# HyeonwooNoh/RAU_VQA

Measured on AMD Instinct MI355X. Metric: QA-pairs/sec fwd+bwd, Ours_SS 8-step RAU, batch 256, 14x14x512, higher is better.
Workload: dtype f32; 1 GPU; Ours_SS 8-step RAU fwd+bwd, 14x14x512, configs[1]; batch_per_gpu=256, global_batch=256, T=26, feature_map=14x14x512, hops=8, parallelism=dp1, collective=none, hop_weights=SS (x nHop), arithmetic=f32 operands, f32 MFMA accumulate, dropout=train mode, Philox masks per step and rank, launch=eager, 3 streams

## Files before the change

### rau_vqa_amd/csrc/common.h

```cpp
#pragma once
#include <hip/hip_runtime.h>
#include <stdint.h>

namespace rau {

typedef float f32x16 __attribute__((ext_vector_type(16)));
typedef float f32x4 __attribute__((ext_vector_type(4)));

constexpr int kWave = 64;

#define RAU_CHAIN_PRIO() __builtin_amdgcn_s_setprio(3)

__device__ __forceinline__ float wave_sum(float v) {
#pragma unroll
  for (int o = 32; o > 0; o >>= 1) v += __shfl_xor(v, o, 64);
  return v;
}
__device__ __forceinline__ float wave_max(float v) {
#pragma unroll
  for (int o = 32; o > 0; o >>= 1) v = fmaxf(v, __shfl_xor(v, o, 64));
  return v;
}
__device__ __forceinline__ float sigmoidf_(float x) { return 1.0f / (1.0f + expf(-x)); }
__device__ __forceinline__ float tanh_fast(float x) {
  const float ax = fabsf(x), x2 = x * x;
  const float p = x * (1.f + x2 * (-0.33333334f + x2 * (0.13333334f + x2 * -0.053968254f)));
  const float t = 1.f - 2.f / (__expf(2.f * ax) + 1.f);
  return ax < 0.125f ? p : copysignf(t, x);
}

__device__ __forceinline__ uint32_t mask_bit(const uint32_t* __restrict__ bits, size_t e) {
  return (bits[e >> 5] >> (e & 31)) & 1u;
}
__device__ __forceinline__ uint32_t mask_nib(const uint32_t* __restrict__ bits, size_t e) {
  return (bits[e >> 5] >> (e & 31)) & 0xFu;
}

__device__ __forceinline__ int xcd_remap(int id, int nwg) {
  const int xcd = id & 7, q = nwg >> 3, r = nwg & 7;
  const int base = xcd < r ? xcd * (q + 1) : r * (q + 1) + (xcd - r) * q;
  return base + (id >> 3);
}

__device__ __forceinline__ float rb16(float x) { return (float)(__bf16)x; }
__device__ __forceinline__ float4 rb16(const float4& v) {
  return make_float4(rb16(v.x), rb16(v.y), rb16(v.z), rb16(v.w));
}

}
```

### rau_vqa_amd/csrc/kernels.h

```cpp
#pragma once
#include <hip/hip_runtime.h>
#include <stddef.h>
#include <stdint.h>

#include "../../include/rau.h"

namespace rau {

constexpr long kMaxSplits = 4096;
constexpr hipError_t kSplitStateError = hipErrorIllegalState;
void split_ws_register(const float* base, size_t floats);
void split_ws_unregister(const float* base);
bool split_span_ok(const float* slab, long nsplit, size_t per_split_floats);

struct LinMode { int bf16 = 0; int deep = 0; };
struct LinOpts {
  const float* bias = nullptr;
  const float* bias2 = nullptr;
  const float* addend = nullptr;
  long add_rs = 0;
  int accumulate = 0;
  int act = 0;
  const float* ymul = nullptr;
  long y_rs = 0;
// ... 170 lines not shown
size_t att_split_part_floats(int nB, int S);
hipError_t att_fwd_split(hipStream_t st, int nB, int M, int A, int S, const float* P,
                         const float* u, const float* ws, const float* bs, const float* zm,
                         const float* I, const float* qf, float* a, float* jv, float* part,
                         const AttPartials& ap = AttPartials());
hipError_t att_bwd_split(hipStream_t st, int nB, int M, int A, int S, const float* I,
                         const float* dj, const float* a, const float* da_lin, const float* ws,
                         float* T_to_dS, float* dz, float* du, float* dwsp, const float* Psrc,
                         const float* u, float* part, int da_ns = 0, int SL = 0,
                         const float* da_add = nullptr);
int att_max_pitch(bool split, int A, int bwd_waves_hint);
inline bool feat_type_ok(int ft) {
  return ft == RAU_FEAT_F32 || ft == RAU_FEAT_F16 || ft == RAU_FEAT_BF16 || ft == RAU_FEAT_E4M3 ||
         ft == RAU_FEAT_E5M2;
}
inline size_t feat_elem_bytes(int ft) {
  return ft == RAU_FEAT_F32 ? 4 : (ft == RAU_FEAT_E4M3 || ft == RAU_FEAT_E5M2) ? 1 : 2;
}
#define RAU_FEAT_TYPE_LIST "RAU_FEAT_F32 | _F16 | _BF16 | _E4M3 | _E5M2"
hipError_t dropout_features(hipStream_t st, int H, size_t per_hop, const void* X,
                            const uint32_t* mask, float mscale, float* xd, size_t mask_e0 = 0,
                            int SL = 0, int Sp = 0, int ft = RAU_FEAT_F32);
hipError_t dropout_features_gen(hipStream_t st, uint64_t seed, uint32_t site, uint32_t step, float p,
                                const uint64_t* key_dev, int H, size_t per_hop, const void* X,
                                float mscale, void* xd, int b16, int ft = RAU_FEAT_F32);
hipError_t dropout_features_b16(hipStream_t st, int H, size_t per_hop, const void* X,
                                const uint32_t* mask, float mscale, void* xd16, int ft = RAU_FEAT_F32);
hipError_t widen_features(hipStream_t st, size_t rows, int SL, int Sp, const void* X, float* out, int ft);
hipError_t expand_features(hipStream_t st, int nB, size_t map_bytes, const void* table, const int32_t* image_of,
                           void* out);
hipError_t bank_gather(hipStream_t st, int n, size_t map_bytes, const void* bank, int32_t capacity,
                       const int32_t* rows, void* out);
hipError_t narrow_features(hipStream_t st, size_t rows, int SL, int Sp, const float* src, void* out, int ft);
hipError_t colsum_acc(hipStream_t st, int rows, int N, const float* X, long ld, float* dst,
                      float* tmp);
hipError_t ce_fwd(hipStream_t st, int nB, int K, int M, const float* logits,
                  const int32_t* labels, const float* mf, const float* wd, const float* bd,
                  float* dl, float* lossrow, int32_t* argmax, float* dopred,
                  const float* part = nullptr, int nsplit = 0, const float* bias = nullptr,
                  float* logits_out = nullptr,
                  int Bper = 0 );
hipError_t loss_reduce(hipStream_t st, int H, int nB, const float* lossrow, float* losses);
constexpr int kMaxAnswers = 16;
hipError_t ce_set_fwd(hipStream_t st, int nB, int K, int M, const float* logits, const int32_t* ids,
                      const float* w, int G, const float* mf, const float* wd, const float* bd, float* dl,
                      float* lossrow, int32_t* argmax, float* dopred, const float* part = nullptr,
                      int nsplit = 0, const float* bias = nullptr, float* logits_out = nullptr, int Bper = 0);
struct Truth {
  const int32_t* labels = nullptr;
  const int32_t* ids = nullptr;
  const float *w = nullptr, *score = nullptr;
  int G = 0;
  bool present() const { return labels || G > 0; }
};
inline const char* criterion_class(const Truth& t) { return t.G > 0 ? "ce_set_fwd" : "ce_fwd"; }
inline hipError_t criterion_head(hipStream_t st, int nB, int K, int M, const float* logits, const Truth& t,
                                 const float* mf, const float* wd, const float* bd, float* dl, float* lossrow,
                                 int32_t* argmax, float* dopred, const float* part = nullptr, int nsplit = 0,
                                 const float* bias = nullptr, float* logits_out = nullptr, int Bper = 0) {
  if (t.G > 0)
    return ce_set_fwd(st, nB, K, M, logits, t.ids, t.w, t.G, mf, wd, bd, dl, lossrow, argmax, dopred, part, nsplit,
                      bias, logits_out, Bper);
  return ce_fwd(st, nB, K, M, logits, t.labels, mf, wd, bd, dl, lossrow, argmax, dopred, part, nsplit, bias,
                logits_out, Bper);
}
hipError_t select_signal(hipStream_t st, int rows, int Bper, int K, int M, const float* dopred,
                         const int32_t* argmax, const Truth& t, const float* selw_dev, const float* wd, float* s,
                         float* add);
// ... 46 lines not shown
```

### rau_vqa_amd/csrc/kernels.hip

```cpp
#include "common.h"
#include <algorithm>
#include <cstdlib>

#include "kernels.h"
#include "philox.h"

namespace rau {

static inline int grid_for(size_t n, int block = 256, int cap = 256 * 8) {
  size_t g = (n + block - 1) / block;
  if (g > (size_t)cap) g = cap;
  if (g < 1) g = 1;
  return (int)g;
}

__global__ void k_fill_masks(uint64_t seed, uint32_t site, uint32_t step, uint32_t thr,
                             size_t nwords, uint32_t* __restrict__ bits,
                             const uint64_t* __restrict__ key) {
  RAU_CHAIN_PRIO();
  if (key) {
    seed = key[0];
    step = (uint32_t)key[1];
  }
  for (size_t w = blockIdx.x * (size_t)blockDim.x + threadIdx.x; w < nwords;
// ... 1542 lines not shown
  LAUNCH_FT(k_widen_features, ft, dim3(grid_for(rows * Sp / 4)), rows * Sp / 4, X,
            reinterpret_cast<float4*>(out));
  return hipGetLastError();
}
#undef LAUNCH_FT

template <typename V>
__global__ __launch_bounds__(256) void k_expand_features(size_t nvec, const V* __restrict__ table,
                                                         const int32_t* __restrict__ image_of,
                                                         V* __restrict__ out) {
  const int b = blockIdx.y;
  const int ib = __builtin_amdgcn_readfirstlane(image_of[b]);
  const V* src = table + (size_t)ib * nvec;
  V* dst = out + (size_t)b * nvec;
  for (size_t i = blockIdx.x * (size_t)blockDim.x + threadIdx.x; i < nvec; i += (size_t)gridDim.x * blockDim.x)
    dst[i] = src[i];
}
hipError_t expand_features(hipStream_t st, int nB, size_t map_bytes, const void* table, const int32_t* image_of,
                           void* out) {
  if (nB <= 0 || !table || !image_of || !out || map_bytes % 8 != 0) return hipErrorInvalidValue;
  const bool v16 = map_bytes % 16 == 0;
  const size_t nvec = map_bytes / (v16 ? 16 : 8);
  const int slices = (int)std::min<size_t>(16, (nvec + 1023) / 1024);
  const dim3 grid(std::max(slices, 1), nB);
  if (v16)
    hipLaunchKernelGGL(k_expand_features<uint4>, grid, dim3(256), 0, st, nvec, static_cast<const uint4*>(table),
                       image_of, static_cast<uint4*>(out));
  else
    hipLaunchKernelGGL(k_expand_features<uint2>, grid, dim3(256), 0, st, nvec, static_cast<const uint2*>(table),
                       image_of, static_cast<uint2*>(out));
  return hipGetLastError();
}

constexpr int kColChunks = 32;
__global__ void k_colsum_stage1(int rows, int N, const float* __restrict__ X, long ld,
                                float* __restrict__ tmp) {
  RAU_CHAIN_PRIO();
  const int n = blockIdx.x * blockDim.x + threadIdx.x;
  if (n >= N) return;
  const int per = (rows + kColChunks - 1) / kColChunks;
  const int r0 = blockIdx.y * per;
  int r1 = r0 + per;
  if (r1 > rows) r1 = rows;
  float acc = 0.f;
  for (int r = r0; r < r1; ++r) acc += X[(size_t)r * ld + n];
  tmp[(size_t)blockIdx.y * N + n] = acc;
}
__global__ __launch_bounds__(256) void k_colsum_stage1_v4(int rows, int N,
                                                         const float* __restrict__ X, long ld,
                                                         float* __restrict__ tmp) {
  __shared__ float4 part[4][64];
  const int l = threadIdx.x & 63, w = threadIdx.x >> 6;
  const int n = (blockIdx.x * 64 + l) * 4;
  const int per = (rows + kColChunks - 1) / kColChunks;
  const int r0 = blockIdx.y * per;
  int r1 = r0 + per;
  if (r1 > rows) r1 = rows;
  float4 a0 = make_float4(0.f, 0.f, 0.f, 0.f), a1 = a0, a2 = a0, a3 = a0;
  if (n < N) {
    const float* p = X + n;
    int r = r0 + w;
    for (; r + 12 < r1; r += 16) {
      const float4 x0 = *reinterpret_cast<const float4*>(p + (size_t)r * ld);
      const float4 x1 = *reinterpret_cast<const float4*>(p + (size_t)(r + 4) * ld);
      const float4 x2 = *reinterpret_cast<const float4*>(p + (size_t)(r + 8) * ld);
      const float4 x3 = *reinterpret_cast<const float4*>(p + (size_t)(r + 12) * ld);
      a0.x += x0.x; a0.y += x0.y; a0.z += x0.z; a0.w += x0.w;
      a1.x += x1.x; a1.y += x1.y; a1.z += x1.z; a1.w += x1.w;
      a2.x += x2.x; a2.y += x2.y; a2.z += x2.z; a2.w += x2.w;
      a3.x += x3.x; a3.y += x3.y; a3.z += x3.z; a3.w += x3.w;
    }
    for (; r < r1; r += 4) {
      const float4 x0 = *reinterpret_cast<const float4*>(p + (size_t)r * ld);
      a0.x += x0.x; a0.y += x0.y; a0.z += x0.z; a0.w += x0.w;
    }
  }
  float4 a;
  a.x = (a0.x + a1.x) + (a2.x + a3.x);
  a.y = (a0.y + a1.y) + (a2.y + a3.y);
  a.z = (a0.z + a1.z) + (a2.z + a3.z);
  a.w = (a0.w + a1.w) + (a2.w + a3.w);
  part[w][l] = a;
  __syncthreads();
  if (w == 0 && n < N) {
    const float4 b = part[1][l], c = part[2][l], d = part[3][l];
    float4 o;
    o.x = (a.x + b.x) + (c.x + d.x);
    o.y = (a.y + b.y) + (c.y + d.y);
    o.z = (a.z + b.z) + (c.z + d.z);
    o.w = (a.w + b.w) + (c.w + d.w);
    *reinterpret_cast<float4*>(tmp + (size_t)blockIdx.y * N + n) = o;
  }
}
__global__ void k_colsum_stage2(int N, const float* __restrict__ tmp, float* __restrict__ dst) {
  RAU_CHAIN_PRIO();
  const int n = blockIdx.x * blockDim.x + threadIdx.x;
  if (n >= N) return;
  float acc = 0.f;
  for (int c = 0; c < kColChunks; ++c) acc += tmp[(size_t)c * N + n];
  dst[n] += acc;
}
hipError_t colsum_acc(hipStream_t st, int rows, int N, const float* X, long ld, float* dst,
                      float* tmp) {
  const bool vec = (N % 4 == 0) && (ld % 4 == 0) && ((reinterpret_cast<uintptr_t>(X) & 15u) == 0) &&
                   rows >= 4 * kColChunks;
  if (vec)
    hipLaunchKernelGGL(k_colsum_stage1_v4, dim3((N + 255) / 256, kColChunks), dim3(256), 0, st,
                       rows, N, X, ld, tmp);
  else
    hipLaunchKernelGGL(k_colsum_stage1, dim3((N + 63) / 64, kColChunks), dim3(64), 0, st, rows, N,
                       X, ld, tmp);
  hipLaunchKernelGGL(k_colsum_stage2, dim3((N + 63) / 64), dim3(64), 0, st, N, tmp, dst);
  return hipGetLastError();
}

__global__ void k_ce_fwd(int nB, int K, int M, const float* __restrict__ logits,
                         const int32_t* __restrict__ labels, const float* __restrict__ mf,
                         const float* __restrict__ wd, const float* __restrict__ bd,
                         float* __restrict__ dl, float* __restrict__ lossrow,
                         int32_t* __restrict__ argmax, float* __restrict__ dopred,
                         const float* __restrict__ part, int nsplit,
                         const float* __restrict__ bias, float* __restrict__ logits_out,
                         int Bper) {
  RAU_CHAIN_PRIO();
  __shared__ float s_val[4];
  __shared__ int s_idx[4];
  __shared__ float s_sum[4];
  const int b = blockIdx.x;
  const int tid = threadIdx.x, l = tid & 63, w = tid >> 6;
  if (nsplit) {
    for (int k = tid; k < K; k += 256) {
      float v = bias[k];
      for (int sp = 0; sp < nsplit; ++sp) v += part[((size_t)sp * nB + b) * K + k];
      logits_out[(size_t)b * K + k] = v;
    }
    __syncthreads();
    logits = logits_out;
  }
  const float* lg = logits + (size_t)b * K;
  float mx = -INFINITY;
  int ai = 0x7fffffff;
  for (int k = tid; k < K; k += 256) {
    const float v = lg[k];
    if (v > mx) { mx = v; ai = k; }
  }
// ... 369 lines not shown
```

### rau_vqa_amd/csrc/rau_ctx.h

```cpp
#pragma once
#include <hip/hip_runtime.h>

#include <algorithm>
#include <array>
#include <cmath>
#include <cstdarg>
#include <cstdio>
#include <cstdlib>
#include <cstring>
#include <numeric>
#include <string>
#include <vector>

#include "../../include/rau.h"
#include "kernels.h"

using namespace rau;

constexpr int kEncHeadTokens = 4;
constexpr int kEncSideChunks = 4;

__attribute__((visibility("hidden"))) int fail(int code, const char* fmt, ...);
#define HIPC(expr)                                                                        \
  do {                                                                                    \
// ... 47 lines not shown
  int ans_G = 0;
  bool regions = false;
};
struct BatchSlot {
  float* feats = nullptr;
  int32_t *tokens = nullptr, *lens_d = nullptr, *labels_d = nullptr;
  int32_t *utok = nullptr, *ustart = nullptr, *upos = nullptr;
  int32_t* image_of_d = nullptr;
  int32_t* bank_idx_d = nullptr;
  float* feats_h = nullptr;
  int32_t *tokens_h = nullptr, *lens_p = nullptr, *labels_h = nullptr;
  int32_t *utok_h = nullptr, *ustart_h = nullptr, *upos_h = nullptr;
  int32_t* image_of_h = nullptr;
  int32_t* bank_idx_h = nullptr;
  int32_t* ans_ids_d = nullptr;
  float *ans_w_d = nullptr, *ans_score_d = nullptr;
  int32_t* ans_h = nullptr;
  bool ans_pending = false;
  int32_t* nreg_d = nullptr;
  int32_t* nreg_h = nullptr;
  bool reg_pending = false;
  hipEvent_t uploaded = nullptr;
  hipEvent_t consumed = nullptr;
  BatchDesc held;
  bool upload_pending = false, consumed_valid = false;
};

struct StreamWs {
  hipStream_t owner = nullptr;
  float* slab = nullptr;
  size_t floats = 0;
  size_t alloc = 0;
  float* coltmp = nullptr;
};

inline Truth truth_of(const BatchSlot& s) {
  return s.held.have_labels ? Truth{s.labels_d, s.ans_ids_d, s.ans_w_d, s.ans_score_d, s.held.ans_G} : Truth{};
}

struct MergeState {
  bool valid = false;
  Truth truth;
  int slot = 0;
  uint64_t serial = 0, fwd = 0;
  bool merged = false;
  uint64_t pred_fwd = 0;
  bool pred_mc = false;
  bool ready = false;
  float *rowf = nullptr, *out = nullptr, *pred = nullptr, *att = nullptr;
  int32_t *rowi = nullptr, *ans = nullptr, *mc = nullptr;
  size_t mc_cap = 0;
  float* score = nullptr;
  void* topk = nullptr;
  int topk_k = 0;
  void invalidate() { valid = merged = false; truth = Truth{}; }
};

struct rau_ctx {
  rau_config cfg;
  int cap = 0;
  int Q;
  int Sp = 0;
  int bf16 = 0;
  hipStream_t st = nullptr;
  hipStream_t st2 = nullptr;
  hipStream_t st3 = nullptr;
// ... 295 lines not shown
```

### rau_vqa_amd/csrc/rau_ctx.hip

```cpp
#include "rau_ctx.h"

static thread_local char g_err[512] = "";
int fail(int code, const char* fmt, ...) {
  va_list ap;
  va_start(ap, fmt);
  vsnprintf(g_err, sizeof(g_err), fmt, ap);
  va_end(ap);
  return code;
}

static int prof_collect(rau_ctx* ctx) {
  if (ctx->precs.empty()) return 0;
  HIPC(hipStreamSynchronize(ctx->st));
  HIPC(hipStreamSynchronize(ctx->st2));
  HIPC(hipStreamSynchronize(ctx->st3));
  if (ctx->stc) HIPC(hipStreamSynchronize(ctx->stc));
  FILE* tl = nullptr;
  if (const char* p = std::getenv("RAU_PROF_TIMELINE")) tl = std::fopen(p, "a");
  for (auto& r : ctx->precs) {
    float ms = 0.f;
    hipEventElapsedTime(&ms, r.a, r.b);
    if (tl) {
      float t0 = 0.f;
      hipEventElapsedTime(&t0, ctx->precs[0].a, r.a);
// ... 407 lines not shown
  CK(dalloc(ctx, &ctx->losses_d, (size_t)H));
  CK(dalloc(ctx, &ctx->hopw_d, (size_t)2 * H));
  {
    hipError_t eh = hipHostMalloc((void**)&ctx->hopw_h, (size_t)4 * H * sizeof(float), hipHostMallocDefault);
    if (eh != hipSuccess) {
      rau_destroy(ctx);
      return fail(RAU_ERR_NOMEM, "hipHostMalloc(hop weights): %s", hipGetErrorString(eh));
    }
  }
  CK(dalloc(ctx, &ctx->argmax_d, HB));
  CK(dalloc(ctx, &ctx->dpre, HB * M));
  CK(dalloc(ctx, &ctx->dhn, HB * R));
  CK(dalloc(ctx, &ctx->dg4, HB * 4 * R));
  for (int i = 0; i < 2; ++i) {
    CK(dalloc(ctx, &ctx->dcn[i], (size_t)B * R));
    CK(dalloc(ctx, &ctx->dhp[i], (size_t)B * R));
  }
  CK(dalloc(ctx, &ctx->dj, HB * M));
  CK(dalloc(ctx, &ctx->da_lin, (size_t)B * S));
  CK(dalloc(ctx, &ctx->dz, HB * S));
  CK(dalloc(ctx, &ctx->du, HB * A));
  CK(dalloc(ctx, &ctx->dwsp, HB * A));
  CK(dalloc(ctx, &ctx->dZ, HB * M * S));
  CK(dalloc(ctx, &ctx->dqt, HB * M));
  CK(dalloc(ctx, &ctx->dQD, HB * Q));
  CK(dalloc(ctx, &ctx->dq, (size_t)B * Q));
  for (StreamWs* w : stream_ws(ctx)) {
    CK(dalloc(ctx, &w->slab, w->floats));
    w->alloc = w->floats;
    split_ws_register(w->slab, w->floats);
  }
  {
    const int widest = std::max({4 * R, 4 * Rq, K, M, S, A, Q});
    CK(dalloc(ctx, &ctx->ws_side.coltmp, (size_t)32 * widest));
    CK(dalloc(ctx, &ctx->ws_bulk.coltmp, (size_t)32 * widest));
    CK(dalloc(ctx, &ctx->dbi_part, (size_t)H * B * M));
    CK(dalloc(ctx, &ctx->tmpS, (size_t)S));
  }
  CK(dalloc(ctx, &ctx->dG1, TB * 4 * Rq));
  CK(dalloc(ctx, &ctx->dG2, TB * 4 * Rq));
  CK(dalloc(ctx, &ctx->dwe, TB * E));
  for (int L = 0; L < 2; ++L) {
    CK(dalloc(ctx, &ctx->edc[L][0], (size_t)B * Rq));
    CK(dalloc(ctx, &ctx->edc[L][1], (size_t)B * Rq));
  }
  CK(dalloc(ctx, &ctx->dkey, (size_t)2, false));
  CK(dalloc(ctx, &ctx->npart, (size_t)1024));
  CK(dalloc(ctx, &ctx->norms_d, (size_t)4));
#undef CK
  {
    hipError_t es = hipStreamSynchronize(ctx->st);
    if (es != hipSuccess) {
      rau_destroy(ctx);
      return fail(RAU_ERR_DEVICE, "rau_create sync: %s", hipGetErrorString(es));
    }
  }
  *out = ctx;
  return RAU_OK;
}

void rau_destroy(rau_ctx* ctx) {
  if (!ctx) return;
  rau_comm_destroy(ctx);
  if (ctx->st_comm) hipStreamDestroy(ctx->st_comm);
  if (ctx->evC) hipEventDestroy(ctx->evC);
  if (ctx->st) hipStreamSynchronize(ctx->st);
  if (ctx->st2) hipStreamSynchronize(ctx->st2);
  if (ctx->st3) hipStreamSynchronize(ctx->st3);
// ... 849 lines not shown
  const size_t BRq = (size_t)B * Rq;
  ctx->fwd_done = false;

  if (!ctx->capturing) {
    if (int rc = upload_hop_weights(ctx, hop_w, select_w)) return rc;
  }
  if (ctx->dpre_fwd && !sel)
    RUN("scale_hops", 0, (double)H * B * (K + M + R) * 8,
        scale_hops3(st, H, ctx->hopw_d, (size_t)B * K, ctx->dl, (size_t)B * M, ctx->dpre, (size_t)B * R, ctx->dhn));
  else
    RUN("scale_hops", 0, (double)H * B * K * 8, scale_hops(st, H, (size_t)B * K, ctx->hopw_d, ctx->dl));

  int HA = 0;
  for (int h = 0; h < H; ++h)
    if (hop_w[h] != 0.f || (sel && select_w[h] != 0.f)) HA = h + 1;

  const uint32_t* m_mf = mk(RAU_MASK_MF);
  if (sel)
    RUN("select_signal", 0, (double)HA * B * M * 4,
        select_signal(st, HA * B, B, K, M, ctx->dopred, ctx->argmax_d, t, ctx->hopw_d + H, ctx->do_pred.W, ctx->sel_s,
                      ctx->sel_add));
  if (HA > 0 && (!ctx->dpre_fwd || sel)) {
    LinOpts o = lin_opts(ctx, ctx->ws_chain);
    if (sel) { o.addend = ctx->sel_add; o.add_rs = M; }
    o.emask = m_mf;
    o.emask_e0 = 0;
    o.emscale = sc(RAU_MASK_MF);
    RUN("head_dgrad", gflop(HA * B, M, K), 0,
        gemm_nn(st, HA * B, M, K, ctx->dl, K, ctx->cls.W, M, ctx->dpre, M, o));
    const LinOpts o2 = lin_opts(ctx, ctx->ws_chain);
    RUN("head_dgrad", gflop(HA * B, R, M), 0,
        gemm_nn(st, HA * B, R, M, ctx->dpre, M, ctx->lstm_out.W, R, ctx->dhn, R, o2));
  }
  const float* dc_next = nullptr;
  float* dh_part = nullptr;
  int dh_part_ns = 0;
  ctx->ds16_step = ctx->dS16 && !ctx->I_shared && !ctx->att_split && conv_dz_fused_ok(S, M, ctx->bf16);
  struct Ds16Reset { rau_ctx* c; ~Ds16Reset() { c->ds16_step = false; } } ds16_reset{ctx};
  bool dq_side = false;
  int dq_rows_left = HA;
  for (int h = HA - 1; h >= 0; --h) {
    float* dc_out = ctx->dcn[h & 1];
    {
      HopGrad g{};
      g.dl = ctx->dl + (size_t)h * B * K;
      g.dc_next = dc_next;
      g.dh_next = nullptr;
      g.dc_out = dc_out;
      g.dh_out = nullptr;
      g.dpre_ready = 1;
      g.dhn_all = ctx->dhn;
      g.dh_part = dh_part;
      g.dh_part_ns = dh_part_ns;
      g.dh_part_out = &dh_part;
      g.dh_part_ns_out = &dh_part_ns;
      g.ev_conv_ready = (gsz[h] && (seam_mask() & 2)) ? ctx->evK[h] : nullptr;
      g.dh_prev_dead = h == 0;
      if (int rc = hop_backward(ctx, h, ctx->cc + (size_t)h * BR_,
                                ctx->I + (ctx->I_shared ? 0 : (size_t)h * BM_ * S), g))
        return rc;
    }
    dc_next = dc_out;
    if (gsz[h] && h > 0 && side_split(ctx)) {
      const int nh = std::min(h + gsz[h], HA) - h;
      HIPC(hipEventRecord(ctx->evK[h], st));
      HIPC(hipStreamWaitEvent(ctx->st3, ctx->evK[h], 0));
// ... 23 lines not shown
                                 ctx->att_i.W, ctx->dj + hb * M,
                                 ctx->a + hb * S, ctx->I + hb * M * S,
                                 ctx->xd16 ? (float*)((uint16_t*)ctx->dZ + hb * M * S) : ctx->dZ + hb * M * S,
                                 ctx->dbi_part + hb * M, ctx->xd16 ? 1 : 0, ctx->bf16, ctx->ds16_step ? 1 : 0,
                                 chain_bound(ctx) ? 1 : 0));
        else
          RUNS(sb, "conv_att_dgrad", gflop(M, (double)nH * S, A),
               ((double)nH * A * S + 2.0 * nH * M * S) * 4,
               conv_att_dgrad(sb, nH, M, S, A, ctx->T + hb * A * S, ctx->att_i.W, ctx->dj + hb * M,
                              ctx->a + hb * S, ctx->dZ + hb * M * S, ctx->bf16));
        {
          if (ctx->ds16_step)
            RUNS(sb, "conv_att_wgrad", gflop(A, M, (double)nH * S),
                 (double)nH * A * S * 2 + (double)nH * M * S * 4,
                 conv_att_wgrad_ds16(sb, nH, M, S, A, (const uint16_t*)ctx->dS16 + hb * A * S,
                                     ctx->I + hb * M * S, ctx->att_i.dW, slab_b));
          else
          RUNS(sb, "conv_att_wgrad", gflop(A, M, (double)nH * S),
               ((double)nH * A * S + (double)nH * M * S) * 4,
               conv_att_wgrad(sb, nH, M, S, A, ctx->T + hb * A * S, ctx->I + hb * M * S,
                              ctx->att_i.dW, slab_b, ctx->bf16));
        }
        if (ctx->xd16 && dzf)
          RUNS(sb, "conv_embed_wgrad", gflop(M, D, (double)nH * S),
               (double)nH * M * S * 2 + (double)nH * D * S * 2,
               conv_embed_wgrad_b16(sb, nH, D, S, M, (const uint16_t*)ctx->dZ + hb * M * S,
                                    (const uint16_t*)ctx->xd16 + hb * D * S, ctx->i_embed.dW, slab_b));
        else
          RUNS(sb, "conv_embed_wgrad", gflop(M, D, (double)nH * S),
               ((double)nH * M * S * (dzf ? 1 : 2) + (double)nH * D * S) * 4,
               conv_embed_wgrad(sb, nH, D, S, M, ctx->dZ + hb * M * S, ctx->I + hb * M * S,
                                  ctx->xd + hb * D * S, ctx->i_embed.dW, slab_b, ctx->bf16,
                                  ctx->i_embed.db, dzf));
        if (dzf && h == 0)
          RUNS(sb, "colsum", 0, (double)HA * B * M * 4,
               colsum_acc(sb, HA * B, M, ctx->dbi_part, M, ctx->i_embed.db, ctx->ws_bulk.coltmp));
      } else {
        for (int hh2 = 0; hh2 < HA; ++hh2) {
          float* Th2 = ctx->T + (size_t)hh2 * B * A * S;
          float* dZh = ctx->dZ + (size_t)hh2 * BM_ * S;
          RUNS(sb, "conv_att_dgrad", gflop(M, (double)B * S, A), ((double)B * A * S + 2.0 * BM_ * S) * 4,
               conv_att_dgrad(sb, B, M, S, A, Th2, ctx->att_i.W, ctx->dj + (size_t)hh2 * BM_,
                              ctx->a + (size_t)hh2 * BS_, dZh, ctx->bf16));
          RUNS(sb, "conv_att_wgrad", gflop(A, M, (double)B * S), ((double)B * A * S + BM_ * S) * 4,
               conv_att_wgrad(sb, B, M, S, A, Th2, ctx->I, ctx->att_i.dW, slab_b, ctx->bf16));
          RUNS(sb, "conv_embed_wgrad", gflop(M, D, (double)B * S), (BM_ * S + (double)B * D * S) * 4,
               conv_embed_wgrad(sb, B, D, S, M, dZh, ctx->I, ctx->xw, ctx->i_embed.dW, slab_b,
                                ctx->bf16, ctx->i_embed.db));
        }
      }
    }
  }
  {
    const LinOpts o = lin_opts(ctx, ctx->ws_chain);
    if (dq_rows_left > 0)
      RUN("q_proj_dgrad", gflop(dq_rows_left * B, Q, M), 0,
          gemm_nn(st, dq_rows_left * B, Q, M, ctx->dqt, M, ctx->q_proj.W, Q, ctx->dQD, Q, o));
    if (dq_side) HIPC(hipStreamWaitEvent(st, ctx->evDq, 0));
    RUN("dq_reduce", 0, (double)HA * B * Q * 4,
        dq_reduce(st, HA, (size_t)B * Q, ctx->dQD, m_q, sc(RAU_MASK_Q), ctx->dq));
  }
  {
    hipStream_t sb = ctx->st2;
    HIPC(hipEventRecord(ctx->evD, sb));
  }
  HIPC(hipEventRecord(ctx->evW, st));
  static const int wg_env = [] { const char* e = std::getenv("RAU_WG_BULK"); return e ? std::atoi(e) : -1; }();
  const int wg_bulk = side_split(ctx) ? 0 : wg_env >= 0 ? wg_env : (chain_bound(ctx) ? 0 : 1);
  auto mult_wgrads = [&]() -> int {
    const StreamWs& ws = (wg_bulk & 1) ? ctx->ws_bulk : ctx->ws_side;
    hipStream_t sw = ws.owner;
    HIPC(hipStreamWaitEvent(sw, ctx->evW, 0));
    const int rows = HA * B;
    if (rows == 0) {
      HIPC(hipEventRecord(ctx->evM3, sw));
      return 0;
    }
    {
      TnProblem pr[13];
      const int np = mult_wgrad_problems(ctx, pr);
      double fl = 0;
      for (int i = 0; i < np; ++i) fl += gflop(pr[i].M, pr[i].N, rows);
      RUNS(sw, "wgrad_gemm", fl, 0, gemm_tn_group_acc(sw, pr, np, rows, ws.slab, ws.floats, lin_mode(ctx).bf16));
    }
    if (sel)
      RUNS(sw, "select_wgrad", 2.0 * rows * (M + 1), (double)rows * M * 4,
           select_wgrad(sw, rows, M, ctx->sel_s, ctx->mf, ctx->do_pred.dW, ctx->do_pred.db));
    RUNS(sw, "colsum", 0, (double)rows * A * 4, colsum_acc(sw, rows, A, ctx->dwsp, A, ctx->att_score.dW, ws.coltmp));
    HIPC(hipMemsetAsync(ctx->tmpS, 0, S * sizeof(float), sw));
    RUNS(sw, "colsum", 0, (double)rows * S * 4, colsum_acc(sw, rows, SL, ctx->dz, S, ctx->tmpS, ws.coltmp));
    RUNS(sw, "colsum", 0, S * 4.0, colsum_acc(sw, SL, 1, ctx->tmpS, 1, ctx->att_score.db, ws.coltmp));
    RUNS(sw, "colsum", 0, (double)rows * A * 4, colsum_acc(sw, rows, A, ctx->du, A, ctx->att_i.db, ws.coltmp));
    HIPC(hipEventRecord(ctx->evM3, sw));
    return 0;
  };
  if (int rc = mult_wgrads()) return rc;

  if (TL > 0) {
    const int rows = TL * B;
    const size_t G4 = (size_t)B * 4 * Rq;
    auto enc_wgrads = [&](int t_lo, int t_hi, hipEvent_t ev) -> int {
      if (t_hi <= t_lo) return 0;
      const StreamWs& ws = (wg_bulk & 2) ? ctx->ws_bulk : ctx->ws_side;
      hipStream_t sw = ws.owner;
      HIPC(hipEventRecord(ev, st));
      HIPC(hipStreamWaitEvent(sw, ev, 0));
      const size_t r0 = (size_t)t_lo * B;
      const int nr = (t_hi - t_lo) * B;
      TnProblem pr[13];
      const int np = enc_wgrad_problems(ctx, r0, pr);
      double fl = 0;
      for (int i = 0; i < np; ++i) fl += gflop(pr[i].M, pr[i].N, nr);
      RUNS(sw, "wgrad_gemm", fl, 0, gemm_tn_group_acc(sw, pr, np, nr, ws.slab, ws.floats, lin_mode(ctx).bf16));
      return 0;
    };
    const int hi = TL;
    for (int u = TL; u >= 0; --u) {
      const float* Ap[3];
      const float* Wp[3];
      int nb = 0, iq2 = -1, iqx = -1, iq1 = -1;
      if (u >= 1 && u + 1 <= TL) { Ap[nb] = ctx->dG2 + (size_t)u * G4; Wp[nb] = ctx->h2h[1].W; iq2 = nb++; }
      if (u + 1 <= TL) { Ap[nb] = ctx->dG2 + (size_t)u * G4; Wp[nb] = ctx->i2h[1].W; iqx = nb++; }
      if (u + 2 <= TL) { Ap[nb] = ctx->dG1 + (size_t)(u + 1) * G4; Wp[nb] = ctx->h2h[0].W; iq1 = nb++; }
      int nsp = 0;
      if (nb > 0)
// ... 317 lines not shown
```

### rau_vqa_amd/csrc/rau_modules.hip

```cpp
#include "rau_ctx.h"

namespace {

bool aligned16(const void* p) { return (reinterpret_cast<uintptr_t>(p) & 15u) == 0; }

int mod_alloc(rau_ctx* ctx) {
  ctx->mg.valid = false;
  if (ctx->mod_ready) return 0;
  const rau_config& c = ctx->cfg;
  const size_t B = ctx->cap, Q = ctx->Q;
  const size_t wide = std::max<size_t>({(size_t)c.Rq, (size_t)c.R, (size_t)c.M});
#define CK(x) do { if (int rc_ = (x)) return rc_; } while (0)
  CK(dalloc(ctx, &ctx->m_state, (size_t)c.T * B * Q));
  CK(dalloc(ctx, &ctx->m_dstate, (size_t)c.T * B * Q));
  for (int i = 0; i < 4; ++i) CK(dalloc(ctx, &ctx->m_tmp[i], B * wide));
  CK(dalloc(ctx, &ctx->m_dq, (size_t)c.H * B * Q));
  CK(dalloc(ctx, &ctx->m_dc, (size_t)c.H * B * c.R));
  CK(dalloc(ctx, &ctx->m_dh, (size_t)c.H * B * c.R));
  CK(dalloc(ctx, &ctx->m_add, B * c.M));
  CK(dalloc(ctx, &ctx->m_s, B));
  CK(dalloc(ctx, &ctx->m_zero, B * std::max<size_t>(Q, (size_t)c.R)));
  CK(dalloc(ctx, &ctx->m_loss, (size_t)c.H));
  if (ctx->Sp != c.S) {
    CK(dalloc(ctx, &ctx->m_Xp, B * c.D * ctx->Sp));
// ... 317 lines not shown
  const size_t BM_ = (size_t)B * M, BS_ = (size_t)B * S, BR_ = (size_t)B * R;
  if (S != SL) {
    if (!resident) {
      if (int rc = repitch(ctx, ctx->m_Xp, S, X, SL, (size_t)B * D)) return rc;
      X = ctx->m_Xp;
    }
    if (d_attprob) {
      HIPC(hipMemsetAsync(ctx->m_da, 0, BS_ * sizeof(float), st));
      if (int rc = repitch(ctx, ctx->m_da, S, d_attprob, SL, B)) return rc;
      d_attprob = ctx->m_da;
    }
  }
  const float* Ih = ctx->I + (size_t)h * BM_ * S;
  const float* mfh = ctx->mf + (size_t)h * BM_;
  float* Th = ctx->T + (size_t)h * B * A * S;
  float* dZh = ctx->dZ + (size_t)h * BM_ * S;
  const float* xin = m.x ? ctx->xd + (size_t)h * B * D * S : X;

  HopGrad g{};
  g.dl = d_logits;
  g.dc_next = d_c;
  g.dh_next = d_h;
  g.da_out = d_attprob;
  g.dc_out = ctx->m_dc + (size_t)h * BR_;
  g.dh_out = ctx->m_dh + (size_t)h * BR_;
  if (d_do_pred) {
    RUN("dopred_bwd", 0, 0, sigmoid_bwd(st, B, d_do_pred, ctx->dopred + (size_t)h * B, ctx->m_s));
    RUN("dopred_bwd", 0, 0, row_scale(st, B, M, ctx->m_s, nullptr, ctx->do_pred.W, ctx->m_add));
    g.dmf_add = ctx->m_add;
  }
  if (int rc = hop_backward(ctx, h, c_prev, Ih, g)) return rc;
  if (d_do_pred) {
    RUN("dopred_bwd", 0, 0, row_scale(st, B, M, ctx->m_s, mfh, nullptr, ctx->m_add));
    RUN("colsum", 0, 0, colsum_acc(st, B, M, ctx->m_add, M, ctx->do_pred.dW, ctx->ws_side.coltmp));
    RUN("colsum", 0, 0, colsum_acc(st, B, 1, ctx->m_s, 1, ctx->do_pred.db, ctx->ws_side.coltmp));
  }
  RUN("conv_att_dgrad", gflop(M, (double)B * S, A), ((double)B * A * S + 2.0 * BM_ * S) * 4,
      conv_att_dgrad(st, B, M, S, A, Th, ctx->att_i.W, ctx->dj + (size_t)h * BM_,
                     ctx->a + (size_t)h * BS_, dZh, ctx->bf16));
  RUN("conv_att_wgrad", gflop(A, M, (double)B * S), ((double)B * A * S + BM_ * S) * 4,
      conv_att_wgrad(st, B, M, S, A, Th, Ih, ctx->att_i.dW, ctx->ws_bulk.slab, ctx->bf16));
  RUN("conv_embed_wgrad", gflop(M, D, (double)B * S), (BM_ * S + (double)B * D * S) * 4,
      conv_embed_wgrad(st, B, D, S, M, dZh, Ih, xin, ctx->i_embed.dW, ctx->ws_bulk.slab, ctx->bf16,
                       ctx->i_embed.db));
  float* dqo = ctx->m_dq + (size_t)h * B * Q;
  {
    LinOpts o = lin_opts(ctx, ctx->ws_chain);
    o.emask = m.q;
    o.emask_e0 = (size_t)h * B * Q;
    o.emscale = m.s_q;
    RUN("q_proj_dgrad", gflop(B, Q, M), 0,
        gemm_nn(st, B, Q, M, ctx->dqt + (size_t)h * BM_, M, ctx->q_proj.W, Q, dqo, Q, o));
  }
  if (d_X) {
    if (!ctx->m_dX) {
      if (int rc = dalloc(ctx, &ctx->m_dX, (size_t)ctx->cap * D * S)) return rc;
      if (int rc = dalloc(ctx, &ctx->m_dZ, (size_t)ctx->cap * M * S)) return rc;
    }
    RUN("mul_dtanh", 0, BM_ * S * 12.0, mul_dtanh(st, BM_ * S, dZh, Ih, ctx->m_dZ));
    RUN("conv_embed_dgrad", gflop(D, (double)B * S, M), (BM_ * S + (double)B * D * S) * 4,
        conv_embed_dgrad(st, B, D, S, M, ctx->m_dZ, ctx->i_embed.W, ctx->m_dX));
    float* dXo = ctx->m_dX;
    if (S != SL) {
      if (!ctx->m_dXd)
        if (int rc = dalloc(ctx, &ctx->m_dXd, (size_t)ctx->cap * D * SL)) return rc;
      if (int rc = repitch(ctx, ctx->m_dXd, SL, ctx->m_dX, S, (size_t)B * D)) return rc;
      dXo = ctx->m_dXd;
    }
    if (m.x)
      RUN("apply_mask", 0, (double)B * D * SL * 8,
          apply_mask(st, (size_t)B * D * SL, (size_t)B * D * SL, dXo, m.x, m.s_x, dXo,
                     (size_t)h * B * D * SL));
    *d_X = dXo;
  }
  const size_t h4 = (size_t)h * B * 4 * R;
  if (int rc = lin_wgrad(ctx, ctx->cls, d_logits, mfh, M)) return rc;
  if (int rc = lin_wgrad(ctx, ctx->lstm_out, ctx->dpre + (size_t)h * BM_, ctx->hh + (size_t)(h + 1) * BR_, R)) return rc;
  if (int rc = lin_wgrad(ctx, ctx->lstm_i2h, ctx->dg4 + h4, ctx->j + (size_t)h * BM_, M)) return rc;
  if (int rc = lin_wgrad(ctx, ctx->lstm_h2h, ctx->dg4 + h4, h_prev, R)) return rc;
  if (int rc = lin_wgrad(ctx, ctx->feat_attprob, ctx->dj + (size_t)h * BM_, ctx->a + (size_t)h * BS_, S)) return rc;
  if (int rc = lin_wgrad(ctx, ctx->att_mem, ctx->dz + (size_t)h * BS_, h_prev, R, true, S)) return rc;
  if (int rc = lin_wgrad(ctx, ctx->att_q, ctx->du + (size_t)h * B * A, ctx->qf + (size_t)h * BM_, M)) return rc;
  if (int rc = lin_wgrad(ctx, ctx->q_proj, ctx->dqt + (size_t)h * BM_, ctx->qd + (size_t)h * B * Q, Q)) return rc;
  if (int rc = lin_wgrad(ctx, ctx->h_proj, ctx->dqt + (size_t)h * BM_, h_prev, R)) return rc;
  RUN("colsum", 0, (double)B * A * 4,
      colsum_acc(st, B, A, ctx->dwsp + (size_t)h * B * A, A, ctx->att_score.dW, ctx->ws_side.coltmp));
  HIPC(hipMemsetAsync(ctx->tmpS, 0, S * sizeof(float), st));
  RUN("colsum", 0, (double)B * S * 4, colsum_acc(st, B, SL, ctx->dz + (size_t)h * BS_, S, ctx->tmpS, ctx->ws_side.coltmp));
  RUN("colsum", 0, S * 4.0, colsum_acc(st, SL, 1, ctx->tmpS, 1, ctx->att_score.db, ctx->ws_side.coltmp));
  RUN("colsum", 0, (double)B * A * 4,
      colsum_acc(st, B, A, ctx->du + (size_t)h * B * A, A, ctx->att_i.db, ctx->ws_side.coltmp));
  if (d_q) *d_q = dqo;
  if (d_c_prev) *d_c_prev = g.dc_out;
  if (d_h_prev) *d_h_prev = g.dh_out;
  return RAU_OK;
}

static int criterion(rau_ctx* ctx, int h, const float* logits, const Truth& t, float* loss, float scale,
                     float** d_logits) {
  const rau_config& c = ctx->cfg;
  float* dl = ctx->dl + (size_t)h * c.B * c.K;
  RUN(criterion_class(t), 0, (double)c.B * c.K * 12,
      criterion_head(ctx->st, c.B, c.K, c.M, logits, t, nullptr, nullptr, nullptr, dl,
                     ctx->lossrow + (size_t)h * c.B, ctx->argmax_d + (size_t)h * c.B, nullptr));
  if (d_logits) {
    if (scale != 1.f)
      RUN("scale_hops", 0, (double)c.B * c.K * 8, scale_inplace(ctx->st, (size_t)c.B * c.K, scale, dl));
    *d_logits = dl;
    return RAU_OK;
  }
  RUN("loss_reduce", 0, 0, loss_reduce(ctx->st, 1, c.B, ctx->lossrow + (size_t)h * c.B, ctx->m_loss + h));
  if (!loss) return RAU_OK;
  HIPC(hipMemcpyAsync(loss, ctx->m_loss + h, sizeof(float), hipMemcpyDeviceToHost, ctx->st));
  HIPC(hipStreamSynchronize(ctx->st));
  return RAU_OK;
}

int rau_criterion_forward(rau_ctx* ctx, int h, const float* logits, const int32_t* labels_dev, float* loss) {
  NEED(ctx && logits, "null argument");
  NEED(h >= 0 && h < ctx->cfg.H, "rau_criterion_forward: h=%d out of [0,%d)", h, ctx->cfg.H);
  if (int rc = mod_alloc(ctx)) return rc;
  const Truth t = labels_dev ? Truth{labels_dev} : truth_of(cur_batch(ctx));
  if (!t.present()) return fail(RAU_ERR_STATE, "rau_criterion_forward: no labels");
  return criterion(ctx, h, logits, t, loss, 1.f, nullptr);
// ... 32 lines not shown
```

Measured before the change: 27680 QA-pairs/s.

## Fuse two-stage column sum into one kernel with last-block reduction

Result: no change. 27620 QA-pairs/s (-0.2%).

```diff
diff --git a/rau_vqa_amd/csrc/common.h b/rau_vqa_amd/csrc/common.h
--- a/rau_vqa_amd/csrc/common.h
+++ b/rau_vqa_amd/csrc/common.h
@@ -20,6 +20,24 @@
 #pragma unroll
   for (int o = 32; o > 0; o >>= 1) v = fmaxf(v, __shfl_xor(v, o, 64));
   return v;
+}
+__device__ __forceinline__ bool last_arrival(unsigned* cnt, unsigned total, int* s_flag) {
+  asm volatile("s_waitcnt vmcnt(0)" ::: "memory");
+  __syncthreads();
+  if (threadIdx.x == 0) {
+    __builtin_amdgcn_fence(__ATOMIC_RELEASE, "agent");
+    asm volatile("s_waitcnt vmcnt(0)" ::: "memory");
+    const unsigned ticket = __hip_atomic_fetch_add(cnt, 1u, __ATOMIC_RELAXED, __HIP_MEMORY_SCOPE_AGENT);
+    const int last = ticket == total - 1;
+    if (last) {
+      __hip_atomic_store(cnt, 0u, __ATOMIC_RELAXED, __HIP_MEMORY_SCOPE_AGENT);
+      __builtin_amdgcn_fence(__ATOMIC_ACQUIRE, "agent");
+      asm volatile("s_waitcnt vmcnt(0)" ::: "memory");
+    }
+    *s_flag = last;
+  }
+  __syncthreads();
+  return *s_flag != 0;
 }
 __device__ __forceinline__ float sigmoidf_(float x) { return 1.0f / (1.0f + expf(-x)); }
 __device__ __forceinline__ float tanh_fast(float x) {
diff --git a/rau_vqa_amd/csrc/kernels.h b/rau_vqa_amd/csrc/kernels.h
--- a/rau_vqa_amd/csrc/kernels.h
+++ b/rau_vqa_amd/csrc/kernels.h
@@ -226,8 +226,9 @@
 hipError_t bank_gather(hipStream_t st, int n, size_t map_bytes, const void* bank, int32_t capacity,
                        const int32_t* rows, void* out);
 hipError_t narrow_features(hipStream_t st, size_t rows, int SL, int Sp, const float* src, void* out, int ft);
+constexpr int kColChunks = 32;
 hipError_t colsum_acc(hipStream_t st, int rows, int N, const float* X, long ld, float* dst,
-                      float* tmp);
+                      float* tmp, unsigned* cnt, int accumulate = 1);
 hipError_t ce_fwd(hipStream_t st, int nB, int K, int M, const float* logits,
                   const int32_t* labels, const float* mf, const float* wd, const float* bd,
                   float* dl, float* lossrow, int32_t* argmax, float* dopred,
diff --git a/rau_vqa_amd/csrc/kernels.hip b/rau_vqa_amd/csrc/kernels.hip
--- a/rau_vqa_amd/csrc/kernels.hip
+++ b/rau_vqa_amd/csrc/kernels.hip
@@ -1598,85 +1598,77 @@
   return hipGetLastError();
 }
 
-constexpr int kColChunks = 32;
-__global__ void k_colsum_stage1(int rows, int N, const float* __restrict__ X, long ld,
-                                float* __restrict__ tmp) {
-  RAU_CHAIN_PRIO();
-  const int n = blockIdx.x * blockDim.x + threadIdx.x;
-  if (n >= N) return;
+__global__ __launch_bounds__(256) void k_colsum(int rows, int N, const float* __restrict__ X, long ld,
+                                                float* __restrict__ dst, float* __restrict__ tmp,
+                                                unsigned* __restrict__ cnt, int vec, int accumulate) {
+  __shared__ float4 part[4][64];
+  __shared__ int is_last;
+  const int tile = blockIdx.x, chunk = blockIdx.y;
   const int per = (rows + kColChunks - 1) / kColChunks;
-  const int r0 = blockIdx.y * per;
+  const int r0 = chunk * per;
   int r1 = r0 + per;
   if (r1 > rows) r1 = rows;
-  float acc = 0.f;
-  for (int r = r0; r < r1; ++r) acc += X[(size_t)r * ld + n];
-  tmp[(size_t)blockIdx.y * N + n] = acc;
-}
-__global__ __launch_bounds__(256) void k_colsum_stage1_v4(int rows, int N,
-                                                         const float* __restrict__ X, long ld,
-                                                         float* __restrict__ tmp) {
-  __shared__ float4 part[4][64];
-  const int l = threadIdx.x & 63, w = threadIdx.x >> 6;
-  const int n = (blockIdx.x * 64 + l) * 4;
-  const int per = (rows + kColChunks - 1) / kColChunks;
-  const int r0 = blockIdx.y * per;
-  int r1 = r0 + per;
-  if (r1 > rows) r1 = rows;
-  float4 a0 = make_float4(0.f, 0.f, 0.f, 0.f), a1 = a0, a2 = a0, a3 = a0;
-  if (n < N) {
-    const float* p = X + n;
-    int r = r0 + w;
-    for (; r + 12 < r1; r += 16) {
-      const float4 x0 = *reinterpret_cast<const float4*>(p + (size_t)r * ld);
-      const float4 x1 = *reinterpret_cast<const float4*>(p + (size_t)(r + 4) * ld);
-      const float4 x2 = *reinterpret_cast<const float4*>(p + (size_t)(r + 8) * ld);
-      const float4 x3 = *reinterpret_cast<const float4*>(p + (size_t)(r + 12) * ld);
-      a0.x += x0.x; a0.y += x0.y; a0.z += x0.z; a0.w += x0.w;
-      a1.x += x1.x; a1.y += x1.y; a1.z += x1.z; a1.w += x1.w;
-      a2.x += x2.x; a2.y += x2.y; a2.z += x2.z; a2.w += x2.w;
-      a3.x += x3.x; a3.y += x3.y; a3.z += x3.z; a3.w += x3.w;
-    }
-    for (; r < r1; r += 4) {
-      const float4 x0 = *reinterpret_cast<const float4*>(p + (size_t)r * ld);
-      a0.x += x0.x; a0.y += x0.y; a0.z += x0.z; a0.w += x0.w;
-    }
-  }
-  float4 a;
-  a.x = (a0.x + a1.x) + (a2.x + a3.x);
-  a.y = (a0.y + a1.y) + (a2.y + a3.y);
-  a.z = (a0.z + a1.z) + (a2.z + a3.z);
-  a.w = (a0.w + a1.w) + (a2.w + a3.w);
-  part[w][l] = a;
-  __syncthreads();
-  if (w == 0 && n < N) {
-    const float4 b = part[1][l], c = part[2][l], d = part[3][l];
-    float4 o;
-    o.x = (a.x + b.x) + (c.x + d.x);
-    o.y = (a.y + b.y) + (c.y + d.y);
-    o.z = (a.z + b.z) + (c.z + d.z);
-    o.w = (a.w + b.w) + (c.w + d.w);
-    *reinterpret_cast<float4*>(tmp + (size_t)blockIdx.y * N + n) = o;
-  }
-}
-__global__ void k_colsum_stage2(int N, const float* __restrict__ tmp, float* __restrict__ dst) {
-  RAU_CHAIN_PRIO();
-  const int n = blockIdx.x * blockDim.x + threadIdx.x;
-  if (n >= N) return;
-  float acc = 0.f;
-  for (int c = 0; c < kColChunks; ++c) acc += tmp[(size_t)c * N + n];
-  dst[n] += acc;
+  if (vec) {
+    const int l = threadIdx.x & 63, w = threadIdx.x >> 6;
+    const int n = (tile * 64 + l) * 4;
+    float4 a0 = make_float4(0.f, 0.f, 0.f, 0.f), a1 = a0, a2 = a0, a3 = a0;
+    if (n < N) {
+      const float* p = X + n;
+      int r = r0 + w;
+      for (; r + 12 < r1; r += 16) {
+        const float4 x0 = *reinterpret_cast<const float4*>(p + (size_t)r * ld);
+        const float4 x1 = *reinterpret_cast<const float4*>(p + (size_t)(r + 4) * ld);
+        const float4 x2 = *reinterpret_cast<const float4*>(p + (size_t)(r + 8) * ld);
+        const float4 x3 = *reinterpret_cast<const float4*>(p + (size_t)(r + 12) * ld);
+        a0.x += x0.x; a0.y += x0.y; a0.z += x0.z; a0.w += x0.w;
+        a1.x += x1.x; a1.y += x1.y; a1.z += x1.z; a1.w += x1.w;
+        a2.x += x2.x; a2.y += x2.y; a2.z += x2.z; a2.w += x2.w;
+        a3.x += x3.x; a3.y += x3.y; a3.z += x3.z; a3.w += x3.w;
+      }
+      for (; r < r1; r += 4) {
+        const float4 x0 = *reinterpret_cast<const float4*>(p + (size_t)r * ld);
+        a0.x += x0.x; a0.y += x0.y; a0.z += x0.z; a0.w += x0.w;
+      }
+    }
+    float4 a;
+    a.x = (a0.x + a1.x) + (a2.x + a3.x);
+    a.y = (a0.y + a1.y) + (a2.y + a3.y);
+    a.z = (a0.z + a1.z) + (a2.z + a3.z);
+    a.w = (a0.w + a1.w) + (a2.w + a3.w);
+    part[w][l] = a;
+    __syncthreads();
+    if (w == 0 && n < N) {
+      const float4 b = part[1][l], c = part[2][l], d = part[3][l];
+      float4 o;
+      o.x = (a.x + b.x) + (c.x + d.x);
+      o.y = (a.y + b.y) + (c.y + d.y);
+      o.z = (a.z + b.z) + (c.z + d.z);
+      o.w = (a.w + b.w) + (c.w + d.w);
+      *reinterpret_cast<float4*>(tmp + (size_t)chunk * N + n) = o;
+    }
+  } else {
+    const int n = tile * 256 + threadIdx.x;
+    if (n < N) {
+      float acc = 0.f;
+      for (int r = r0; r < r1; ++r) acc += X[(size_t)r * ld + n];
+      tmp[(size_t)chunk * N + n] = acc;
+    }
+  }
+  if (!last_arrival(cnt, gridDim.x * gridDim.y, &is_last)) return;
+  for (int n = threadIdx.x; n < N; n += 256) {
+    float acc = 0.f;
+    for (int c = 0; c < kColChunks; ++c) acc += tmp[(size_t)c * N + n];
+    if (accumulate) dst[n] += acc;
+    else dst[n] = acc;
+  }
 }
 hipError_t colsum_acc(hipStream_t st, int rows, int N, const float* X, long ld, float* dst,
-                      float* tmp) {
-  const bool vec = (N % 4 == 0) && (ld % 4 == 0) && ((reinterpret_cast<uintptr_t>(X) & 15u) == 0) &&
-                   rows >= 4 * kColChunks;
-  if (vec)
-    hipLaunchKernelGGL(k_colsum_stage1_v4, dim3((N + 255) / 256, kColChunks), dim3(256), 0, st,
-                       rows, N, X, ld, tmp);
-  else
-    hipLaunchKernelGGL(k_colsum_stage1, dim3((N + 63) / 64, kColChunks), dim3(64), 0, st, rows, N,
-                       X, ld, tmp);
-  hipLaunchKernelGGL(k_colsum_stage2, dim3((N + 63) / 64), dim3(64), 0, st, N, tmp, dst);
+                      float* tmp, unsigned* cnt, int accumulate) {
+  if (N <= 0) return hipSuccess;
+  const int vec = (N % 4 == 0) && (ld % 4 == 0) && ((reinterpret_cast<uintptr_t>(X) & 15u) == 0) &&
+                  rows >= 4 * kColChunks;
+  hipLaunchKernelGGL(k_colsum, dim3((N + 255) / 256, kColChunks), dim3(256), 0, st, rows, N, X, ld, dst, tmp,
+                     cnt, vec, accumulate);
   return hipGetLastError();
 }
 
diff --git a/rau_vqa_amd/csrc/rau_ctx.h b/rau_vqa_amd/csrc/rau_ctx.h
--- a/rau_vqa_amd/csrc/rau_ctx.h
+++ b/rau_vqa_amd/csrc/rau_ctx.h
@@ -103,6 +103,7 @@
   size_t floats = 0;
   size_t alloc = 0;
   float* coltmp = nullptr;
+  unsigned* colcnt = nullptr;
 };
 
 inline Truth truth_of(const BatchSlot& s) {
diff --git a/rau_vqa_amd/csrc/rau_ctx.hip b/rau_vqa_amd/csrc/rau_ctx.hip
--- a/rau_vqa_amd/csrc/rau_ctx.hip
+++ b/rau_vqa_amd/csrc/rau_ctx.hip
@@ -463,8 +463,12 @@
   }
   {
     const int widest = std::max({4 * R, 4 * Rq, K, M, S, A, Q});
-    CK(dalloc(ctx, &ctx->ws_side.coltmp, (size_t)32 * widest));
-    CK(dalloc(ctx, &ctx->ws_bulk.coltmp, (size_t)32 * widest));
+    for (StreamWs* w : {&ctx->ws_side, &ctx->ws_bulk}) {
+      CK(dalloc(ctx, &w->coltmp, (size_t)kColChunks * widest));
+      float* f = nullptr;
+      CK(dalloc(ctx, &f, 4));
+      w->colcnt = reinterpret_cast<unsigned*>(f);
+    }
     CK(dalloc(ctx, &ctx->dbi_part, (size_t)H * B * M));
     CK(dalloc(ctx, &ctx->tmpS, (size_t)S));
   }
@@ -1380,6 +1384,9 @@
     RUN("head_dgrad", gflop(HA * B, R, M), 0,
         gemm_nn(st, HA * B, R, M, ctx->dpre, M, ctx->lstm_out.W, R, ctx->dhn, R, o2));
   }
+  static const int wg_env = [] { const char* e = std::getenv("RAU_WG_BULK"); return e ? std::atoi(e) : -1; }();
+  const int wg_bulk = side_split(ctx) ? 0 : wg_env >= 0 ? wg_env : (chain_bound(ctx) ? 0 : 1);
+  bool dbi_pending = false;
   const float* dc_next = nullptr;
   float* dh_part = nullptr;
   int dh_part_ns = 0;
@@ -1469,9 +1476,14 @@
                conv_embed_wgrad(sb, nH, D, S, M, ctx->dZ + hb * M * S, ctx->I + hb * M * S,
                                   ctx->xd + hb * D * S, ctx->i_embed.dW, slab_b, ctx->bf16,
                                   ctx->i_embed.db, dzf));
-        if (dzf && h == 0)
-          RUNS(sb, "colsum", 0, (double)HA * B * M * 4,
-               colsum_acc(sb, HA * B, M, ctx->dbi_part, M, ctx->i_embed.db, ctx->ws_bulk.coltmp));
+        if (dzf && h == 0) {
+          if (wg_bulk & 1)
+            dbi_pending = true;
+          else
+            RUNS(sb, "colsum", 0, (double)HA * B * M * 4,
+                 colsum_acc(sb, HA * B, M, ctx->dbi_part, M, ctx->i_embed.db, ctx->ws_bulk.coltmp,
+                            ctx->ws_bulk.colcnt));
+        }
       } else {
         for (int hh2 = 0; hh2 < HA; ++hh2) {
           float* Th2 = ctx->T + (size_t)hh2 * B * A * S;
@@ -1502,8 +1514,6 @@
     HIPC(hipEventRecord(ctx->evD, sb));
   }
   HIPC(hipEventRecord(ctx->evW, st));
-  static const int wg_env = [] { const char* e = std::getenv("RAU_WG_BULK"); return e ? std::atoi(e) : -1; }();
-  const int wg_bulk = side_split(ctx) ? 0 : wg_env >= 0 ? wg_env : (chain_bound(ctx) ? 0 : 1);
   auto mult_wgrads = [&]() -> int {
     const StreamWs& ws = (wg_bulk & 1) ? ctx->ws_bulk : ctx->ws_side;
     hipStream_t sw = ws.owner;
@@ -1513,6 +1523,16 @@
       HIPC(hipEventRecord(ctx->evM3, sw));
       return 0;
     }
+    if (dbi_pending)
+      RUNS(sw, "colsum", 0, (double)rows * M * 4,
+           colsum_acc(sw, rows, M, ctx->dbi_part, M, ctx->i_embed.db, ws.coltmp, ws.colcnt));
+    RUNS(sw, "colsum", 0, (double)rows * A * 4,
+         colsum_acc(sw, rows, A, ctx->dwsp, A, ctx->att_score.dW, ws.coltmp, ws.colcnt));
+    RUNS(sw, "colsum", 0, (double)rows * S * 4,
+         colsum_acc(sw, rows, SL, ctx->dz, S, ctx->tmpS, ws.coltmp, ws.colcnt, 0));
+    RUNS(sw, "colsum", 0, S * 4.0, colsum_acc(sw, SL, 1, ctx->tmpS, 1, ctx->att_score.db, ws.coltmp, ws.colcnt));
+    RUNS(sw, "colsum", 0, (double)rows * A * 4,
+         colsum_acc(sw, rows, A, ctx->du, A, ctx->att_i.db, ws.coltmp, ws.colcnt));
     {
       TnProblem pr[13];
       const int np = mult_wgrad_problems(ctx, pr);
@@ -1523,11 +1543,6 @@
     if (sel)
       RUNS(sw, "select_wgrad", 2.0 * rows * (M + 1), (double)rows * M * 4,
            select_wgrad(sw, rows, M, ctx->sel_s, ctx->mf, ctx->do_pred.dW, ctx->do_pred.db));
-    RUNS(sw, "colsum", 0, (double)rows * A * 4, colsum_acc(sw, rows, A, ctx->dwsp, A, ctx->att_score.dW, ws.coltmp));
-    HIPC(hipMemsetAsync(ctx->tmpS, 0, S * sizeof(float), sw));
-    RUNS(sw, "colsum", 0, (double)rows * S * 4, colsum_acc(sw, rows, SL, ctx->dz, S, ctx->tmpS, ws.coltmp));
-    RUNS(sw, "colsum", 0, S * 4.0, colsum_acc(sw, SL, 1, ctx->tmpS, 1, ctx->att_score.db, ws.coltmp));
-    RUNS(sw, "colsum", 0, (double)rows * A * 4, colsum_acc(sw, rows, A, ctx->du, A, ctx->att_i.db, ws.coltmp));
     HIPC(hipEventRecord(ctx->evM3, sw));
     return 0;
   };
diff --git a/rau_vqa_amd/csrc/rau_modules.hip b/rau_vqa_amd/csrc/rau_modules.hip
--- a/rau_vqa_amd/csrc/rau_modules.hip
+++ b/rau_vqa_amd/csrc/rau_modules.hip
@@ -373,8 +373,8 @@
   if (int rc = hop_backward(ctx, h, c_prev, Ih, g)) return rc;
   if (d_do_pred) {
     RUN("dopred_bwd", 0, 0, row_scale(st, B, M, ctx->m_s, mfh, nullptr, ctx->m_add));
-    RUN("colsum", 0, 0, colsum_acc(st, B, M, ctx->m_add, M, ctx->do_pred.dW, ctx->ws_side.coltmp));
-    RUN("colsum", 0, 0, colsum_acc(st, B, 1, ctx->m_s, 1, ctx->do_pred.db, ctx->ws_side.coltmp));
+    RUN("colsum", 0, 0, colsum_acc(st, B, M, ctx->m_add, M, ctx->do_pred.dW, ctx->ws_side.coltmp, ctx->ws_side.colcnt));
+    RUN("colsum", 0, 0, colsum_acc(st, B, 1, ctx->m_s, 1, ctx->do_pred.db, ctx->ws_side.coltmp, ctx->ws_side.colcnt));
   }
   RUN("conv_att_dgrad", gflop(M, (double)B * S, A), ((double)B * A * S + 2.0 * BM_ * S) * 4,
       conv_att_dgrad(st, B, M, S, A, Th, ctx->att_i.W, ctx->dj + (size_t)h * BM_,
@@ -424,13 +424,16 @@
   if (int rc = lin_wgrad(ctx, ctx->att_q, ctx->du + (size_t)h * B * A, ctx->qf + (size_t)h * BM_, M)) return rc;
   if (int rc = lin_wgrad(ctx, ctx->q_proj, ctx->dqt + (size_t)h * BM_, ctx->qd + (size_t)h * B * Q, Q)) return rc;
   if (int rc = lin_wgrad(ctx, ctx->h_proj, ctx->dqt + (size_t)h * BM_, h_prev, R)) return rc;
-  RUN("colsum", 0, (double)B * A * 4,
-      colsum_acc(st, B, A, ctx->dwsp + (size_t)h * B * A, A, ctx->att_score.dW, ctx->ws_side.coltmp));
-  HIPC(hipMemsetAsync(ctx->tmpS, 0, S * sizeof(float), st));
-  RUN("colsum", 0, (double)B * S * 4, colsum_acc(st, B, SL, ctx->dz + (size_t)h * BS_, S, ctx->tmpS, ctx->ws_side.coltmp));
-  RUN("colsum", 0, S * 4.0, colsum_acc(st, SL, 1, ctx->tmpS, 1, ctx->att_score.db, ctx->ws_side.coltmp));
-  RUN("colsum", 0, (double)B * A * 4,
-      colsum_acc(st, B, A, ctx->du + (size_t)h * B * A, A, ctx->att_i.db, ctx->ws_side.coltmp));
+  {
+    const StreamWs& ws = ctx->ws_side;
+    RUN("colsum", 0, (double)B * A * 4,
+        colsum_acc(st, B, A, ctx->dwsp + (size_t)h * B * A, A, ctx->att_score.dW, ws.coltmp, ws.colcnt));
+    RUN("colsum", 0, (double)B * S * 4,
+        colsum_acc(st, B, SL, ctx->dz + (size_t)h * BS_, S, ctx->tmpS, ws.coltmp, ws.colcnt, 0));
+    RUN("colsum", 0, S * 4.0, colsum_acc(st, SL, 1, ctx->tmpS, 1, ctx->att_score.db, ws.coltmp, ws.colcnt));
+    RUN("colsum", 0, (double)B * A * 4,
+        colsum_acc(st, B, A, ctx->du + (size_t)h * B * A, A, ctx->att_i.db, ws.coltmp, ws.colcnt));
+  }
   if (d_q) *d_q = dqo;
   if (d_c_prev) *d_c_prev = g.dc_out;
   if (d_h_prev) *d_h_prev = g.dh_out;
```
